# kekley/octree_pathtracing

Hardware: AMD Instinct MI355X
Metric: Mrays/sec at 1920×1080×256spp; achieved HBM GB/s vs roofline at 1/2/4/8 GPUs (higher is better)
Workload: dtype f32

## Files before the change

include/octpt.h:

```cpp
#ifndef OCTPT_H
#define OCTPT_H

#include <stddef.h>
#include <stdint.h>

#ifdef __cplusplus
extern "C" {
#endif

#define OCTPT_ABI_VERSION 4u

typedef int32_t octpt_status;
#define OCTPT_OK 0
#define OCTPT_ERR_INVALID_ARG 1
#define OCTPT_ERR_OOM 2
#define OCTPT_ERR_DEVICE 3
#define OCTPT_NOT_READY 4
#define OCTPT_ERR_UNSUPPORTED 5
#define OCTPT_CANCELLED 6
#define OCTPT_ERR_INTERNAL 7

typedef struct octpt_ctx octpt_ctx;
typedef struct octpt_frame octpt_frame;
typedef struct octpt_octree octpt_octree;
// ... 122 lines not shown
#define OCTPT_STAT_ESVO_STEPS 2
#define OCTPT_STAT_SPHERE_TESTS 3
#define OCTPT_STAT_CUBOID_TESTS 4
#define OCTPT_STAT_SHADE_EVENTS 5
#define OCTPT_STAT_TEXEL_READS 6
#define OCTPT_STAT_BLOCK_TESTS 7
#define OCTPT_STAT_ISSUED_BYTES 8
#define OCTPT_STAT_COUNT 9
typedef struct octpt_stats {
    uint64_t paths, segments, esvo_steps, sphere_tests, cuboid_tests, shade_events, texel_reads;
    uint64_t launches;
    double kernel_ms;
    uint64_t extend_launches, shade_launches;
    double extend_ms, shade_ms;
    double build_ms;
    uint64_t block_tests;
    uint64_t issued_bytes;
    uint64_t drain[OCTPT_STAT_COUNT];
    uint64_t pool_slots;
    uint64_t chunk_items;
    uint64_t wave_allocs;
    uint64_t beam_restarts;
    uint64_t hit_check_failures;
} octpt_stats;

uint32_t octpt_abi_version(void);
int32_t octpt_device_count(void);
octpt_status octpt_create(int32_t device, octpt_ctx **out);
octpt_status octpt_create_multi(const int32_t *devices, uint32_t n, octpt_ctx **out);
uint32_t octpt_device_entries(const octpt_ctx *ctx);
void octpt_destroy(octpt_ctx *ctx);
const char *octpt_last_error(const octpt_ctx *ctx);

octpt_status octpt_scene_upload(octpt_ctx *ctx, const octpt_scene_desc *scene);
octpt_status octpt_scene_build_device(octpt_ctx *ctx, const octpt_scene_desc *scene, uint32_t flags);
octpt_status octpt_set_camera(octpt_ctx *ctx, const octpt_camera *camera);
octpt_status octpt_get_camera(const octpt_ctx *ctx, octpt_camera *camera);

octpt_status octpt_render(octpt_ctx *ctx, const octpt_render_params *p, float *accum_rgba, uint8_t *out_rgba8);

octpt_status octpt_render_device(octpt_ctx *ctx, const octpt_render_params *p, float *d_accum,
                                 uint32_t *d_seg_count, void *hip_stream);

octpt_status octpt_render_async(octpt_ctx *ctx, const octpt_render_params *p, float *accum_rgba,
                                uint8_t *out_rgba8, octpt_frame **out_frame);
octpt_status octpt_frame_poll(octpt_frame *frame);
// ... 271 lines not shown
```

octree_pathtracing_amd/_lib.py:

```python
from __future__ import annotations

import ctypes as C
import os
from pathlib import Path

LIB_DIR = Path(__file__).resolve().parent / "lib"
LIB_PATH = LIB_DIR / "liboctpt.so"

OCTPT_ABI_VERSION = 4

OK = 0
ERR_INVALID_ARG = 1
ERR_OOM = 2
ERR_DEVICE = 3
NOT_READY = 4
ERR_UNSUPPORTED = 5
CANCELLED = 6
ERR_INTERNAL = 7

TEXTURE_COLOR = 0
TEXTURE_IMAGE = 1
RENDER_SHARD_COMPACT = 0x1
RENDER_MEGAKERNEL = 0x2
RENDER_KERNEL_TIMING = 0x4
# ... 210 lines not shown
    _fields_ = [("width", C.c_uint32), ("height", C.c_uint32), ("flags", C.c_uint32)]


class FinalParams(C.Structure):
    _fields_ = [("adaptive", AdaptiveParamsEx), ("filter", DenoiseVarianceParams)]


TILE = 8


STAT_NAMES = ("paths", "segments", "esvo_steps", "sphere_tests", "cuboid_tests", "shade_events", "texel_reads",
              "block_tests", "issued_bytes")
STAT_COUNT = len(STAT_NAMES)


class Stats(C.Structure):
    _fields_ = [("paths", C.c_uint64), ("segments", C.c_uint64), ("esvo_steps", C.c_uint64),
                ("sphere_tests", C.c_uint64), ("cuboid_tests", C.c_uint64), ("shade_events", C.c_uint64),
                ("texel_reads", C.c_uint64), ("launches", C.c_uint64), ("kernel_ms", C.c_double),
                ("extend_launches", C.c_uint64), ("shade_launches", C.c_uint64), ("extend_ms", C.c_double),
                ("shade_ms", C.c_double), ("build_ms", C.c_double), ("block_tests", C.c_uint64),
                ("issued_bytes", C.c_uint64), ("drain", C.c_uint64 * STAT_COUNT), ("pool_slots", C.c_uint64),
                ("chunk_items", C.c_uint64), ("wave_allocs", C.c_uint64), ("beam_restarts", C.c_uint64),
                ("hit_check_failures", C.c_uint64)]

    def as_dict(self) -> dict:
        d = {name: getattr(self, name) for name, _ in self._fields_}
        d["drain"] = dict(zip(STAT_NAMES, list(self.drain)))
        return d


class OctreeView(C.Structure):
    _fields_ = [("octants", C.c_void_p), ("octant_count", C.c_uint32), ("root", C.c_uint32), ("depth", C.c_uint32),
                ("leaf_first", C.c_void_p), ("leaf_count", C.c_void_p), ("leaf_table_size", C.c_uint32),
                ("leaf_prims", C.c_void_p), ("leaf_prim_count", C.c_uint32)]


_vp, _u32, _i32, _f = C.c_void_p, C.c_uint32, C.c_int32, C.c_float
SIGNATURES = {
    "octpt_abi_version": (_u32, []),
    "octpt_device_count": (_i32, []),
    "octpt_create": (_i32, [_i32, C.POINTER(_vp)]),
    "octpt_create_multi": (_i32, [_vp, _u32, C.POINTER(_vp)]),
    "octpt_device_entries": (_u32, [_vp]),
    "octpt_destroy": (None, [_vp]),
    "octpt_last_error": (C.c_char_p, [_vp]),
    "octpt_scene_upload": (_i32, [_vp, C.POINTER(SceneDesc)]),
# ... 109 lines not shown
```

octree_pathtracing_amd/csrc/octpt_api.cpp:

```cpp
#include <hip/hip_runtime.h>

#include <algorithm>
#include <atomic>
#include <chrono>
#include <cmath>
#include <cstdlib>
#include <thread>
#include <cstdio>
#include <cstring>
#include <new>
#include <string>
#include <memory>
#include <vector>

#include "../../include/octpt.h"
#include "octpt_internal.h"
#include "octpt_mask.h"
#include "octpt_reproject.h"

using namespace octpt;

namespace {

constexpr uint32_t kCounterRing = 256;
constexpr uint64_t kMaxChunkPaths = 1ull << 31;
constexpr uint64_t kDefaultChunkPaths = 1ull << 29;
#ifndef OCTPT_LOOKAHEAD
#define OCTPT_LOOKAHEAD 3
#endif
constexpr uint32_t kLookahead = OCTPT_LOOKAHEAD;
constexpr uint32_t kDefaultPool = 512u << 20;
constexpr uint32_t kMaxPool = 1u << 30;
constexpr uint32_t kMinPool = 1u << 20;
constexpr uint32_t kDefaultRefill = 0;
constexpr uint32_t kDefaultDrainRays = 4096;

uint32_t env_u32(const char *name, uint32_t dflt) {
    const char *v = std::getenv(name);
    if (!v || !*v) return dflt;
    const long x = std::strtol(v, nullptr, 10);
    return x > 0 ? (uint32_t)x : dflt;
}

struct EventPair {
    hipEvent_t start, stop;
};

template <class T>
struct DevBuf {
    T *p = nullptr;
    size_t n = 0;
};

}

struct octpt_ctx {
    int device = 0;
// ... 7 lines not shown
    octpt_camera cam{};
    DevCamera C{};
    uint32_t *d_counters = nullptr;
    std::vector<uint2> h_subs;
    uint2 *d_subs = nullptr;
    size_t subs_cap = 0;
    float *d_beam = nullptr;
    size_t beam_cap = 0;
    uint32_t launch_seq = 0;
    unsigned long long *d_stats = nullptr;
    uint8_t *d_lut_byte = nullptr;
    float *d_lut_float = nullptr;
    std::vector<EventPair> pending;
    double kernel_ms = 0.0;
    uint64_t launches = 0;
    bool ktiming = false;
    std::vector<std::pair<int, EventPair>> kpending;
    std::vector<EventPair> ev_pool;
    double kern_ms[2] = {0.0, 0.0};
    uint64_t kern_n[2] = {0, 0};
    float build_ms = 0.0f;
    BuildScratch build_scratch;
    int blocks_per_cu_cache[kMaxDepth + 1] = {0};
    int extend_bpc_cache[kMaxDepth + 1][4] = {};
    int shade_bpc_cache[2][2][3] = {};
    bool lean_scene = false;
    bool no_lean = false;
    WaveBuffers wb{};
    size_t pool = 0, color_cap = 0, nee_pool = 0;
    void *nee_alloc = nullptr;
    std::vector<void *> wave_allocs;
    void *color_alloc = nullptr;
    size_t wave_bytes = 0, mem_limit = 0;
    std::vector<std::pair<void *, size_t>> wave_sizes;
    uint64_t wave_allocs_n = 0;
    bool oom_warned = false;
    uint32_t *h_count = nullptr;
    uint32_t *d_count = nullptr;
    hipEvent_t count_ev[kLookahead + 1] = {};
    uint32_t pool_cap = kDefaultPool, refill = kDefaultRefill;
    bool beam = true;
    uint32_t drain_rays = kDefaultDrainRays;
    bool drain_models = false;
    uint64_t chunk_cap = kDefaultChunkPaths;
    octpt_frame *inflight = nullptr;
    std::vector<octpt_ctx *> sub;
    float4 *m_acc = nullptr;
    uint32_t *m_seg = nullptr;
    size_t m_acc_cap = 0, m_seg_cap = 0;
    float4 *dn_frame[2] = {nullptr, nullptr};
    size_t dn_cap[2] = {0, 0};
    std::vector<uint32_t> h_order;
    uint32_t order_w = 0, order_h = 0;
    uint32_t *d_order = nullptr, *d_order_pos = nullptr;
    uint64_t scene_gen = 0, camera_gen = 0, order_gen = 0;
    struct BeamKey {
        uint64_t scene = 0, camera = 0, order = 0;
        uint64_t list = 0;
        uint32_t w = 0, h = 0, shard_index = 0, shard_count = 0;
        bool valid = false;
        bool operator==(const BeamKey &o) const {
            return valid && o.valid && scene == o.scene && camera == o.camera && order == o.order && list == o.list &&
                   w == o.w && h == o.h && shard_index == o.shard_index && shard_count == o.shard_count;
// ... 742 lines not shown
                         ctx->S.sun.sun_sampling != 0, ctx->S.has_blocks != 0, &part);
        if (st == OCTPT_OK) break;
        if (st != OCTPT_ERR_OOM) return st;
        if (part == kOomColor && chunk_spp > 1 && !R.subs) {
            ctx->chunk_cap = (uint64_t)(chunk_spp / 2) * n_px;
            if (ctx->pool > ctx->chunk_cap) {
                HIP_TRY(ctx, hipDeviceSynchronize());
                free_queues(ctx);
                ctx->pool_cap = (uint32_t)std::max<uint64_t>(kMinPool, std::min<uint64_t>(ctx->pool_cap, ctx->chunk_cap));
            }
        } else if (part == kOomNee && ctx->pool > kMinPool) {
            HIP_TRY(ctx, hipDeviceSynchronize());
            ctx->pool_cap = (uint32_t)std::max<size_t>(kMinPool, ctx->pool / 2);
            free_queues(ctx);
        } else {
            return st;
        }
        if (!ctx->oom_warned)
            std::fprintf(stderr, "octpt: wavefront state did not fit in device memory; chunk %llu items, pool cap %u\n",
                         (unsigned long long)ctx->chunk_cap, ctx->pool_cap);
        ctx->oom_warned = true;
    }
    const size_t pool = (size_t)std::min<uint64_t>(std::min<uint64_t>(ctx->pool_cap, chunk_max), ctx->pool);
    int &bpc = ctx->extend_bpc_cache[ctx->S.depth][ctx->S.has_blocks ? 3 : ctx->S.has_models ? 2 : (ctx->S.has_cuboids ? 1 : 0)];
    if (bpc == 0) bpc = extend_blocks_per_cu(ctx->S);
    const int grid_extend = ctx->num_cu * bpc;
    if (std::getenv("OCTPT_DEBUG"))
        std::fprintf(stderr, "octpt: extend %d blocks/CU x %d CUs (depth %u, cuboids %u, models %u), pool %zu\n", bpc,
                     ctx->num_cu, ctx->S.depth, ctx->S.has_cuboids, ctx->S.has_models, pool);
    const int seg_blocks = (int)(kSegs * 64u / kBlock);
    const uint32_t shade_bpc_env = std::min<uint32_t>(env_u32("OCTPT_SHADE_BPC", 0u), 8u);
    auto grid_shade_of = [&](int mode) {
        int &cached = ctx->shade_bpc_cache[ctx->S.sun.sun_sampling ? 1 : 0]
                                          [shade_lds_tables(ctx->S) ? 1 : 0]
                                          [mode];
        if (cached == 0) cached = shade_blocks_per_cu(ctx->S, mode);
        const int bpc = shade_bpc_env ? (int)shade_bpc_env : cached;
        return (ctx->num_cu * bpc + seg_blocks - 1) / seg_blocks * seg_blocks;
    };
    {
        float none;
        std::memcpy(&none, &kPrimNone, sizeof none);
        ctx->wb.eye = make_float4(ctx->C.eye[0], ctx->C.eye[1], ctx->C.eye[2], none);
    }
    const WaveBuffers &B = ctx->wb;
    const float *beam = nullptr;
    if (ctx->beam) {
        const size_t n_tiles = (size_t)R.beam_tx * ((R.H + kBeamTile - 1) / kBeamTile);
        octpt_ctx::BeamKey key;
        key.scene = ctx->scene_gen;
        key.camera = ctx->camera_gen;
        key.order = ctx->order_gen;
        key.w = R.W;
        key.h = R.H;
        key.shard_index = R.shard_index;
        key.shard_count = R.shard_count;
        key.list = list;
        key.valid = true;
        if (list != 0u) {
// ... 26 lines not shown
        beam = ctx->d_beam;
    }
    for (uint32_t c0 = 0, c1 = 0; c0 < R.spp_count; c0 = c1) {
        c1 = c0 + std::min(chunk_spp, R.spp_count - c0);
        if (R.subs) {
            uint32_t e = c1;
            while (e < R.spp_count && (ctx->h_subs[e].y >> 16) != 0u) --e;
            if (e <= c0) {
                e = c1;
                while (e < R.spp_count && (ctx->h_subs[e].y >> 16) != 0u) ++e;
            }
            c1 = e;
        }
        DevRender Rc = R;
        Rc.spp_start = R.spp_start + c0;
        Rc.spp_count = c1 - c0;
        if (R.subs) Rc.subs = R.subs + c0;
        Rc.beam = beam;
        const uint32_t chunk_items = (uint32_t)((uint64_t)Rc.spp_count * n_px);
        HIP_TRY(ctx, hipMemsetAsync(B.ctrl, 0, kCtrlWords * sizeof(uint32_t), s));
        const uint32_t n_seed = (uint32_t)std::min<uint64_t>(pool, chunk_items);
        const bool regen = n_seed < chunk_items;
        ctx->wb.lean = (!regen && ctx->lean_scene && !ctx->no_lean && !R.subs) ? 1u : 0u;
        const int grid_shade = grid_shade_of(shade_mode(regen, ctx->wb.lean != 0u));
        const bool cam_rec = !regen &&((Rc.W | Rc.H) & (kTile - 1u)) == 0u;
        HIP_TRY(ctx, launch_wf_seed(ctx->C, Rc, B, n_seed, chunk_items, ctx->d_stats, s));
        for (uint32_t it = 0;; ++it) {
            if (cancel && cancel->load()) return fail(ctx, OCTPT_CANCELLED, "render cancelled");
            const uint32_t q = it & 1u;
            EventPair ev{};
            if ((st = ktimer_begin(ctx, s, ev)) != OCTPT_OK) return st;
            HIP_TRY(ctx, launch_wf_extend(ctx->S, B, q, it == 0u && cam_rec, ctx->refill, grid_extend,
                                          ctx->d_stats, s));
            if ((st = ktimer_end(ctx, s, 0, ev)) != OCTPT_OK) return st;
            if ((st = ktimer_begin(ctx, s, ev)) != OCTPT_OK) return st;
            HIP_TRY(ctx, launch_wf_shade(ctx->S, ctx->C, Rc, B, q, chunk_items, it == 0u ? (cam_rec ? 2u : 1u) : 0u,
                                         regen, grid_shade, ctx->d_stats, s));
            if ((st = ktimer_end(ctx, s, 1, ev)) != OCTPT_OK) return st;
            const uint32_t slot = it % (kLookahead + 1);
            HIP_TRY(ctx, launch_wf_snapshot(B, q ^ 1u, ctx->d_count + slot * kCountSpan, s));
            HIP_TRY(ctx, hipEventRecord(ctx->count_ev[slot], s));
            if (it >= kLookahead) {
                const uint32_t old = (it - kLookahead) % (kLookahead + 1);
                HIP_TRY(ctx, hipEventSynchronize(ctx->count_ev[old]));
                const uint32_t *h = ctx->h_count + old * kCountSpan;
                uint64_t queued = 0;
                for (uint32_t k = 0; k < kSegs; ++k) queued += h[k];
                if (queued == 0u) break;
                if (queued <= ctx->drain_rays && (!ctx->S.has_models || ctx->drain_models)) {
                    bool exhausted = true;
                    for (uint32_t k = 0; k < kSegs && exhausted; ++k) {
                        const uint32_t lo = (uint32_t)(((uint64_t)k * chunk_items) / kSegs);
                        const uint32_t hi = (uint32_t)(((uint64_t)(k + 1u) * chunk_items) / kSegs);
                        exhausted = h[kSegs + k] >= hi - lo;
                    }
                    if (exhausted) {
                        const int grid = (int)std::min<uint64_t>((queued + 3) / 4 + 1, (uint64_t)ctx->num_cu * 16u);
                        HIP_TRY(ctx, launch_wf_drain(ctx->S, Rc, B, q ^ 1u, grid, ctx->d_stats, s));
                        break;
                    }
// ... 337 lines not shown
octpt_status octpt_create(int32_t device, octpt_ctx **out) {
    if (!out) return OCTPT_ERR_INVALID_ARG;
    *out = nullptr;
    octpt_ctx *ctx = new (std::nothrow) octpt_ctx();
    if (!ctx) return OCTPT_ERR_OOM;
    auto bail = [&](octpt_status st) {
        octpt_destroy(ctx);
        return st;
    };
    int n = 0;
    if (hipGetDeviceCount(&n) != hipSuccess || n == 0) return bail(OCTPT_ERR_DEVICE);
    if (device < 0 || device >= n) return bail(OCTPT_ERR_INVALID_ARG);
    hipDeviceProp_t prop{};
    if (hipGetDeviceProperties(&prop, device) != hipSuccess) return bail(OCTPT_ERR_DEVICE);
    if (std::strncmp(prop.gcnArchName, "gfx950", 6) != 0) return bail(OCTPT_ERR_DEVICE);
    ctx->device = device;
    ctx->num_cu = prop.multiProcessorCount;
    ctx->pool_cap = std::max<uint32_t>(std::min<uint32_t>(env_u32("OCTPT_POOL", kDefaultPool), kMaxPool), 64u);
    ctx->chunk_cap = std::min<uint64_t>(env_u32("OCTPT_CHUNK", (uint32_t)kDefaultChunkPaths), kMaxChunkPaths);
    const char *refill_env = std::getenv("OCTPT_REFILL");
    ctx->refill = (refill_env && *refill_env)
                      ? std::max<uint32_t>(std::min<uint32_t>(env_u32("OCTPT_REFILL", 16u), 64u), 1u)
                      : kDefaultRefill;
    const char *drain_env = std::getenv("OCTPT_DRAIN_RAYS");
    if (drain_env && *drain_env) ctx->drain_rays = (uint32_t)std::strtoul(drain_env, nullptr, 10);
    const char *beam_env = std::getenv("OCTPT_BEAM");
    ctx->beam = !(beam_env && beam_env[0] == '0');
    const char *lean_env = std::getenv("OCTPT_LEAN");
    ctx->no_lean = lean_env && lean_env[0] == '0';
    ctx->drain_models = env_u32("OCTPT_DRAIN_MODELS", 0u) != 0u;
    ctx->mem_limit = (size_t)env_u32("OCTPT_DEVICE_MEM_LIMIT", 0u) << 20;
    if (hipSetDevice(device) != hipSuccess) return bail(OCTPT_ERR_DEVICE);
    if (hipStreamCreateWithFlags(&ctx->stream, hipStreamNonBlocking) != hipSuccess) return bail(OCTPT_ERR_DEVICE);
    if (hipMalloc(&ctx->d_counters, kCounterRing * sizeof(uint32_t)) != hipSuccess) return bail(OCTPT_ERR_OOM);
    if (hipMalloc(&ctx->d_stats, kStatWords * sizeof(unsigned long long)) != hipSuccess) return bail(OCTPT_ERR_OOM);
    if (hipMemset(ctx->d_stats, 0, kStatWords * sizeof(unsigned long long)) != hipSuccess) return bail(OCTPT_ERR_DEVICE);
    float lf[256];
    uint8_t lb[256];
    make_luts(lf, lb);
    if (hipMalloc(&ctx->d_lut_float, sizeof lf) != hipSuccess) return bail(OCTPT_ERR_OOM);
    if (hipMalloc(&ctx->d_lut_byte, sizeof lb) != hipSuccess) return bail(OCTPT_ERR_OOM);
    if (hipMemcpy(ctx->d_lut_float, lf, sizeof lf, hipMemcpyHostToDevice) != hipSuccess) return bail(OCTPT_ERR_DEVICE);
    if (hipMemcpy(ctx->d_lut_byte, lb, sizeof lb, hipMemcpyHostToDevice) != hipSuccess) return bail(OCTPT_ERR_DEVICE);
    *out = ctx;
    return OCTPT_OK;
}
// ... 1747 lines not shown
            octpt_stats cs{};
            const octpt_status st = octpt_get_stats(c, &cs);
            if (st != OCTPT_OK) return fail(ctx, st, c->err);
            tot.paths += cs.paths;
            tot.segments += cs.segments;
            tot.esvo_steps += cs.esvo_steps;
            tot.sphere_tests += cs.sphere_tests;
            tot.cuboid_tests += cs.cuboid_tests;
            tot.shade_events += cs.shade_events;
            tot.texel_reads += cs.texel_reads;
            tot.extend_launches += cs.extend_launches;
            tot.shade_launches += cs.shade_launches;
            tot.extend_ms += cs.extend_ms;
            tot.shade_ms += cs.shade_ms;
            tot.build_ms = std::max(tot.build_ms, cs.build_ms);
            tot.block_tests += cs.block_tests;
            tot.issued_bytes += cs.issued_bytes;
            for (int k = 0; k < OCTPT_STAT_COUNT; ++k) tot.drain[k] += cs.drain[k];
            tot.pool_slots = std::max(tot.pool_slots, cs.pool_slots);
            tot.chunk_items = std::max(tot.chunk_items, cs.chunk_items);
            tot.wave_allocs += cs.wave_allocs;
            tot.beam_restarts += cs.beam_restarts;
            tot.hit_check_failures += cs.hit_check_failures;
        }
        tot.build_ms = std::max(tot.build_ms, (double)ctx->build_ms);
        tot.launches = ctx->launches;
        tot.kernel_ms = ctx->kernel_ms;
        *out = tot;
        return OCTPT_OK;
    }
    HIP_TRY(ctx, hipSetDevice(ctx->device));
    for (auto &e : ctx->pending) {
        HIP_TRY(ctx, hipEventSynchronize(e.stop));
        float ms = 0.0f;
        HIP_TRY(ctx, hipEventElapsedTime(&ms, e.start, e.stop));
        ctx->kernel_ms += ms;
        (void)hipEventDestroy(e.start);
        (void)hipEventDestroy(e.stop);
    }
    ctx->pending.clear();
    for (auto &ke : ctx->kpending) {
        HIP_TRY(ctx, hipEventSynchronize(ke.second.stop));
        float ms = 0.0f;
        HIP_TRY(ctx, hipEventElapsedTime(&ms, ke.second.start, ke.second.stop));
        ctx->kern_ms[ke.first] += ms;
        ctx->kern_n[ke.first]++;
// ... 30 lines not shown
    }
    out->paths = v[kStatPaths];
    out->segments = v[kStatSegments] - redo_main;
    out->esvo_steps = v[kStatSteps];
    out->sphere_tests = v[kStatSphereTests];
    out->cuboid_tests = v[kStatCuboidTests];
    out->shade_events = v[kStatShade];
    out->texel_reads = v[kStatTexels];
    out->block_tests = v[kStatBlockTests];
    out->issued_bytes = v[kStatIssued];
    out->beam_restarts = redo_main + redo_drain;
    out->hit_check_failures = 0;
    for (uint32_t r = 0; r < 2u * kSegs; ++r) out->hit_check_failures += rows[r * kStatRow + kStatHitCheckWord];
    out->pool_slots = ctx->pool;
    out->chunk_items = ctx->color_cap;
    out->wave_allocs = ctx->wave_allocs_n;
    out->launches = ctx->launches;
    out->kernel_ms = ctx->kernel_ms;
    out->extend_launches = ctx->kern_n[0];
    out->shade_launches = ctx->kern_n[1];
    out->extend_ms = ctx->kern_ms[0];
    out->shade_ms = ctx->kern_ms[1];
    out->build_ms = ctx->build_ms;
    return OCTPT_OK;
}

octpt_status octpt_reset_stats(octpt_ctx *ctx) {
    if (!ctx) return OCTPT_ERR_INVALID_ARG;
    join_inflight(ctx);
    if (is_multi(ctx)) {
        for (octpt_ctx *c : ctx->sub) {
            const octpt_status st = octpt_reset_stats(c);
            if (st != OCTPT_OK) return fail(ctx, st, c->err);
        }
        ctx->kernel_ms = 0.0;
        ctx->launches = 0;
        return OCTPT_OK;
    }
    octpt_stats tmp;
    octpt_status st = octpt_get_stats(ctx, &tmp);
    if (st != OCTPT_OK) return st;
    HIP_TRY(ctx, hipMemset(ctx->d_stats, 0, kStatWords * sizeof(unsigned long long)));
    ctx->kernel_ms = 0.0;
    ctx->launches = 0;
    ctx->kern_ms[0] = ctx->kern_ms[1] = 0.0;
    ctx->kern_n[0] = ctx->kern_n[1] = 0;
    return OCTPT_OK;
}

octpt_status octpt_build_octree_device(octpt_ctx *ctx, const octpt_sphere *spheres, uint32_t ns,
                                       const octpt_cuboid *cuboids, uint32_t nc, uint32_t depth, octpt_octree **out) {
    return octpt_build_octree_device_ex(ctx, spheres, ns, cuboids, nc, depth, 0u, out);
}

octpt_status octpt_build_octree_device_ex(octpt_ctx *ctx, const octpt_sphere *spheres, uint32_t ns,
                                          const octpt_cuboid *cuboids, uint32_t nc, uint32_t depth, uint32_t flags,
                                          octpt_octree **out) {
    if (!ctx) return OCTPT_ERR_INVALID_ARG;
    if (!out) return fail(ctx, OCTPT_ERR_INVALID_ARG, "out NULL");
    if (flags & ~OCTPT_BUILD_COMPACT) return fail(ctx, OCTPT_ERR_INVALID_ARG, "unknown build flags");
    *out = nullptr;
    if (depth < 1 || depth > kMaxDepth) return fail(ctx, OCTPT_ERR_INVALID_ARG, "depth must be in [1, 21]");
    if ((ns && !spheres) || (nc && !cuboids)) return fail(ctx, OCTPT_ERR_INVALID_ARG, "NULL primitive array");
    return build_octree_handle(ctx, out, "octree build", [=](BuiltOctree &t, float &ms) {
        join_inflight(ctx);
        if (pair_bound(spheres, ns, cuboids, nc, depth) > kMaxBuildPairs)
            return fail(ctx, OCTPT_ERR_OOM, "more than 2^31 (cell, primitive) pairs");
        HIP_TRY(ctx, hipSetDevice(ctx->device));
        return run_prim_build(ctx, spheres, ns, cuboids, nc, depth, flags, t, nullptr, ms);
// ... 34 lines not shown
```

octree_pathtracing_amd/csrc/octpt_internal.h:

```cpp
#pragma once
#include <hip/hip_runtime.h>
#include <stdint.h>

#include <memory>
#include <new>
#include <utility>
#include <vector>

#include "../../include/octpt.h"

namespace octpt {

constexpr uint32_t kPrimNone = 0xFFFFFFFFu;
constexpr uint32_t kPrimCuboidBit = 0x80000000u;
constexpr uint32_t kPrimIndexMask = 0x07FFFFFFu;
#ifndef OCTPT_BEAM_TILE
#define OCTPT_BEAM_TILE 2
#endif
constexpr uint32_t kBeamTile = OCTPT_BEAM_TILE;
constexpr uint32_t kTile = 8;
constexpr uint32_t kBlock = 256;
constexpr uint32_t kMaxDepth = 21;
constexpr uint64_t kMaxBuildPairs = 1ull << 31;

// ... 232 lines not shown
    if (compact) {
        caller = i;
        return true;
    }
    const uint32_t t = dealt_tile(order, shard_index + u * shard_count);
    const uint32_t x = (t % tiles_x) * kTile + k % kTile, y = (t / tiles_x) * kTile + k / kTile;
    if (x >= W || y >= H) return false;
    caller = y * W + x;
    return true;
}

hipError_t launch_preview(const DevScene &S, const DevCamera &C, const DevRender &R, float4 *accum,
                          uint32_t *segcount, unsigned long long *stats, hipStream_t stream);
hipError_t launch_render(const DevScene &S, const DevCamera &C, const DevRender &R, float4 *accum,
                         uint32_t *segcount, uint32_t *counter, unsigned long long *stats, int grid,
                         hipStream_t stream);
hipError_t launch_wf_seed(const DevCamera &C, const DevRender &R, const WaveBuffers &B, uint32_t n_seed,
                          uint32_t chunk_items, unsigned long long *stats, hipStream_t stream);
hipError_t launch_wf_extend(const DevScene &S, const WaveBuffers &B, uint32_t q, bool cam, uint32_t refill, int grid,
                            unsigned long long *stats, hipStream_t stream);
hipError_t launch_wf_shade(const DevScene &S, const DevCamera &C, const DevRender &R, const WaveBuffers &B, uint32_t q,
                           uint32_t chunk_items, uint32_t first, bool regen, int grid, unsigned long long *stats,
                           hipStream_t stream);
int shade_blocks_per_cu(const DevScene &S, int mode);
bool shade_lds_tables(const DevScene &S);
hipError_t launch_wf_drain(const DevScene &S, const DevRender &R, const WaveBuffers &B, uint32_t q, int grid,
                           unsigned long long *stats, hipStream_t stream);
hipError_t launch_wf_snapshot(const WaveBuffers &B, uint32_t q, uint32_t *host_out, hipStream_t stream);
hipError_t launch_wf_resolve(const DevRender &R, const WaveBuffers &B, uint32_t chunk_spp, float4 *accum,
                             uint32_t *segcount, float2 *moments, float clamp, hipStream_t stream);
hipError_t launch_adaptive_init(uint32_t n, float4 *accum, float2 *moments, hipStream_t stream);
hipError_t launch_tile_error(uint32_t W, uint32_t H, float luminance_floor, const float2 *moments,
                             const uint32_t *tile_spp, float *error, hipStream_t stream);
hipError_t launch_tile_error_spread(uint32_t W, uint32_t H, float w, const float *error, float *out, hipStream_t stream);
hipError_t launch_sample_variance(uint32_t W, uint32_t H, const float2 *moments, const uint32_t *tile_spp,
                                  const float *depth, const float4 *albedo, float *out, hipStream_t stream);
int extend_blocks_per_cu(const DevScene &S);
hipError_t launch_intersect(const DevScene &S, const float *rays, const uint32_t *last_prim,
                            const float *last_normal, uint32_t n, float *t, uint32_t *prim, float *normal,
                            uint32_t *steps, hipStream_t stream);
hipError_t launch_beam(const DevScene &S, const DevCamera &C, const DevRender &R, float *beam, hipStream_t stream);
hipError_t launch_gbuffer(const DevScene &S, const DevCamera &C, const DevRender &R, const DevAov &out,
                          unsigned long long *stats, hipStream_t stream);
hipError_t launch_denoise_prep(uint32_t W, uint32_t H, const float4 *color, const float4 *albedo, const float *depth,
                               float4 *sig, hipStream_t stream);
hipError_t launch_atrous(const DevDenoise &D, uint32_t iter, bool last, const float4 *src, float4 *dst,
                         hipStream_t stream);
hipError_t launch_temporal(const DevTemporal &T, bool moments, hipStream_t stream);
hipError_t launch_variance(const DevVariance &V, hipStream_t stream);
hipError_t launch_denoise_var_prep(uint32_t W, uint32_t H, const float4 *color, const float *variance,
                                   const float4 *albedo, const float *depth, float4 *sig, hipStream_t stream);
hipError_t launch_atrous_var(const DevDenoiseVar &D, uint32_t iter, bool last, const float4 *src, float4 *dst,
                             hipStream_t stream);
hipError_t launch_tonemap(const float4 *accum, uchar4 *out, uint32_t n, const uint8_t *lut_byte,
                          hipStream_t stream);
hipError_t launch_unshard(uint32_t W, uint32_t H, uint32_t shard_count, const uint32_t *tile_pos, const float4 *shards,
                          uint32_t stride, float4 *frame, hipStream_t stream);
hipError_t launch_multi_stage(const DevRender &R, uint32_t n_dev, uint32_t stride, float4 *accum, uint32_t *seg,
                              float4 *stage_accum, uint32_t *stage_seg, bool to_stage, hipStream_t stream);
int render_blocks_per_cu(uint32_t depth);
// ... 91 lines not shown
```

octree_pathtracing_amd/csrc/octpt_kernels.hip:

```cpp
#include "octpt_internal.h"
#include "octpt_rcp.h"
#include "octpt_reproject.h"

#ifndef OCTPT_RCP_FAST
#define OCTPT_RCP_FAST 1
#endif

namespace octpt {
namespace {

#define RAY_EPSILON 0.00000005f
#define RAY_OFFSET 0.000001f
#define OCTREE_MAX_STEPS 1000u
#define OCTREE_MAX_SCALE 23u
#define OCTREE_EPSILON 1.1920929e-7f
#define MAX_DST_WORLD 1024.0f
#define PI_F 3.14159265358979323846f
#define CELL_TOL 0.001f
#define SUN_MAX_CHANCE 0.9f
#define MAT_FLAG_REFRACTIVE 0x4u
#define MAT_FLAG_SUBSURFACE 0x2u
#define MAX_PATH_SEGMENTS 64u
constexpr uint32_t kBeamIterBits = 10u;
constexpr uint32_t kBeamIterMask = (1u << kBeamIterBits) - 1u;
// ... 1714 lines not shown
    }
    return ok;
}

__global__ __launch_bounds__(kBlock) void wf_seed_kernel(DevCamera C, DevRender R, WaveBuffers B, uint32_t n_seed,
                                                         uint32_t chunk_items, unsigned long long *__restrict__ stats) {
    const uint32_t i = blockIdx.x * kBlock + threadIdx.x;
    const uint32_t seg = (i >> 6) % kSegs;
    Counters cnt = {0u, 0u, 0u, 0u, 0u, 0u, 0u};
    PathState ps;
    bool ok = false;
    uint32_t slot = i;
    if (n_seed == chunk_items) {
        if (blockIdx.x == 0u && threadIdx.x < kSegs)
            B.ctrl[ctr_item(threadIdx.x)] = shard_lo(threadIdx.x + 1u, chunk_items) - shard_lo(threadIdx.x, chunk_items);
        const uint32_t lo = shard_lo(seg, chunk_items), hi = shard_lo(seg + 1u, chunk_items);
        const uint32_t item = lo + (i >> 6) / kSegs * 64u + (i & 63u);
        slot = item;
        if (item < hi) ok = seed_item<true>(C, R, B, slot, item, ps, cnt);
        if (((R.W | R.H) & (kTile - 1u)) == 0u) {
            if (blockIdx.x == 0u && threadIdx.x < kSegs)
                B.ctrl[ctr_count(0u, threadIdx.x)] = shard_lo(threadIdx.x + 1u, chunk_items) - shard_lo(threadIdx.x, chunk_items);
            if (ok) store_cam_ray(B, seg * B.seg_cap + (item - lo), ps);
            if (blockIdx.x == 0u && threadIdx.x == 0u) B.ray0[0][0] = B.eye;
            if (blockIdx.x == 0u && threadIdx.x == 0u) atomicAdd(&stats[kStatPaths], (unsigned long long)chunk_items);
            return;
        }
    } else {
        ItemCursor cur = {seg, true};
        ok = regen<true>(C, R, B, i, i < n_seed, chunk_items, cur, ps, cnt);
    }
    const uint32_t t = wave_ticket(B.ctrl + ctr_count(0u, seg), ok);
    if (ok) store_ray(B, 0u, seg * B.seg_cap + t, slot, ps);
    flush_counters(cnt, stats);
}

#ifndef OCTPT_SPH_WAVES
#define OCTPT_SPH_WAVES 8
#endif
#ifndef OCTPT_BOX_WAVES
#define OCTPT_BOX_WAVES 7
#endif
#ifndef OCTPT_MDL_WAVES
#define OCTPT_MDL_WAVES 6
#endif
#ifndef OCTPT_BLK_WAVES
#define OCTPT_BLK_WAVES 6
#endif
#define OCTPT_EXTEND_WAVES_OF(k)                                                                              \
    ((k) == kPrimsSpheres ? OCTPT_SPH_WAVES                                                                   \
                          : (k) == kPrimsBoxes ? OCTPT_BOX_WAVES : (k) == kPrimsBlocks ? OCTPT_BLK_WAVES : OCTPT_MDL_WAVES)
#ifndef OCTPT_CLAIM
#define OCTPT_CLAIM 64
#endif
constexpr uint32_t kClaim = OCTPT_CLAIM;
static_assert(kSegs % 8u == 0u, "eight XCDs share the segments evenly");
#ifndef OCTPT_THR_LONG
#define OCTPT_THR_LONG 16
#endif
#ifndef OCTPT_THR_SHORT
#define OCTPT_THR_SHORT 32
#endif
#ifndef OCTPT_SHORT_STEPS
#define OCTPT_SHORT_STEPS 48
#endif
constexpr uint32_t kShortRaySteps = OCTPT_SHORT_STEPS;
template <int kPrims>
__global__ __launch_bounds__(kBlock, OCTPT_EXTEND_WAVES_OF(kPrims)) void wf_extend_kernel(DevScene S, WaveBuffers B, uint32_t q, uint32_t refill,
                                                           unsigned long long *__restrict__ stats) {
    extern __shared__ uint2 lds_stack[];
    const Stack stk = stack_of(lds_stack, S.depth);
    const float4 *ray0 = B.ray0[q], *ray1 = B.ray1[q];
    const bool cam = (refill >> 31) != 0u;
    refill &= 0x7FFFFFFFu;
    if (blockIdx.x == 0 && threadIdx.x < kSegs) {
        B.ctrl[ctr_count(q ^ 1u, threadIdx.x)] = 0u;
        B.ctrl[ctr_head(q ^ 1u, threadIdx.x)] = 0u;
    }
    uint32_t seg = __builtin_amdgcn_readfirstlane(((blockIdx.x * kBlock + threadIdx.x) >> 6) % kSegs);
    uint32_t seg_n = B.ctrl[ctr_count(q, seg)];
    if constexpr (kPrims == kPrimsModels) seg_n = __builtin_amdgcn_readfirstlane(seg_n);
    bool rays_left = true;
    uint32_t segs_w = 0u;
    Counters cnt = {0u, 0u, 0u, 0u, 0u, 0u, 0u};
    constexpr uint32_t kIdle = 8u;
    uint32_t pos = 0u;
    TraceRay tr;
    Esvo E;
    E.idx = kIdle;
    bool more = true;
    const uint32_t lane = threadIdx.x & 63u;
    uint32_t c_next = 0u, c_end = 0u, claim_v = 0u;
    uint32_t thr = refill ? refill : OCTPT_THR_LONG;
    if (lane == 0u)
        claim_v = __hip_atomic_fetch_add(B.ctrl + ctr_head(q, seg), kClaim, __ATOMIC_RELAXED, __HIP_MEMORY_SCOPE_AGENT);
    do {
        const bool idle = E.idx >= kIdle;
        const uint64_t im = __ballot(idle);
        if (rays_left && (uint32_t)__popcll(im) >= thr) {
            if (c_next >= c_end) {
                c_next = __builtin_amdgcn_readfirstlane(claim_v);
                c_end = c_next < seg_n ? __builtin_amdgcn_readfirstlane(min(c_next + kClaim, seg_n))
                                       : c_next;
                if (c_next >= c_end) {
                    uint32_t j = lane;
                    if constexpr (kPrims != kPrimsSpheres) asm volatile("" : "+v"(j));
                    const uint64_t m = __ballot(relaxed_load(B.ctrl + ctr_head(q, j)) < B.ctrl[ctr_count(q, j)]);
                    rays_left = m != 0ull;
                    if (rays_left) {
                        seg = __builtin_amdgcn_readfirstlane(first_from(m, seg));
                        seg_n = B.ctrl[ctr_count(q, seg)];
                        if constexpr (kPrims == kPrimsModels) seg_n = __builtin_amdgcn_readfirstlane(seg_n);
                    }
                }
                if (rays_left && lane == 0u)
                    claim_v = __hip_atomic_fetch_add(B.ctrl + ctr_head(q, seg), kClaim,
                                                     __ATOMIC_RELAXED, __HIP_MEMORY_SCOPE_AGENT);
            }
            const uint32_t avail = c_end - c_next;
            if (idle) {
                const uint32_t r = lanes_below(im);
                if (r < avail) {
                    pos = seg * B.seg_cap + c_next + r;
                    const float4 r1 = ray1[pos];
                    const float4 r0 = ray0[cam ? 0u : pos];
                    const float bm = cam ? r1.w : ray_beam(r0, r1);
                    tr = make_trace_ray(S, V(r0.x, r0.y, r0.z), V(r1.x, r1.y, r1.z), ray_last_prim(r0, r1),
                                        (__float_as_uint(r1.w) >> 31) != 0u);
                    esvo_begin(S, tr, E, stk, bm);
                    cnt.steps -= E.iter;
                }
            }
            const uint32_t took = min((uint32_t)__popcll(im), avail);
            segs_w += took;
            c_next += took;
            if (refill == 0u) {
                const bool short_rays = (int64_t)(int32_t)cnt.steps * 64 < (int64_t)kShortRaySteps * segs_w;
                thr = __popcll(__ballot(short_rays)) > 32 ? OCTPT_THR_SHORT : OCTPT_THR_LONG;
            }
        }
        const uint32_t stop_at = __builtin_amdgcn_readfirstlane(rays_left ? thr : 64u);
        if ((uint32_t)__popcll(__ballot(E.idx >= kIdle)) < stop_at) do {
#ifdef OCTPT_PROFILE_LANES
            prof_wave(cnt.p_iters, cnt.p_active, E.idx < kIdle);
#endif
            if (E.idx < kIdle) {
                uint32_t prim = kPrimNone;
#ifndef OCTPT_CHECK_HITS
                if constexpr (kPrims != kPrimsModels) asm("" : "=v"(prim));
#endif
                PrimHit h;
                HIT_POISON(prim, h);
// ... 1011 lines not shown
    if (D.out_variance) D.out_variance[p] = o.w;
    const float alpha = D.color[p].w;
    if (D.albedo && zp != __builtin_inff()) {
        const float4 a = D.albedo[p];
        o.x = o.x * fmaxf(a.x, kDnAlbedoFloor);
        o.y = o.y * fmaxf(a.y, kDnAlbedoFloor);
        o.z = o.z * fmaxf(a.z, kDnAlbedoFloor);
    }
    D.out[p] = make_float4(o.x, o.y, o.z, alpha);
}

}

size_t render_lds_bytes(uint32_t depth) { return (size_t)(depth - 1u) * kBlock * (sizeof(uint2) + sizeof(uint16_t)); }

int render_blocks_per_cu(uint32_t depth) {
    int blocks = 0;
    if (hipOccupancyMaxActiveBlocksPerMultiprocessor(&blocks, reinterpret_cast<const void *>(render_kernel<true, kPrimsModels>),
                                                     kBlock, render_lds_bytes(depth)) != hipSuccess)
        return 1;
    return blocks > 0 ? blocks : 1;
}

static const void *extend_instance(const DevScene &S) {
    if (S.has_blocks) return reinterpret_cast<const void *>(wf_extend_kernel<kPrimsBlocks>);
    if (S.has_models) return reinterpret_cast<const void *>(wf_extend_kernel<kPrimsModels>);
    if (S.has_cuboids) return reinterpret_cast<const void *>(wf_extend_kernel<kPrimsBoxes>);
    return reinterpret_cast<const void *>(wf_extend_kernel<kPrimsSpheres>);
}

int extend_blocks_per_cu(const DevScene &S) {
    int blocks = 0;
    if (hipOccupancyMaxActiveBlocksPerMultiprocessor(&blocks, extend_instance(S), kBlock, render_lds_bytes(S.depth)) !=
        hipSuccess)
        return 1;
    return blocks > 0 ? blocks : 1;
}

hipError_t launch_preview(const DevScene &S0, const DevCamera &C, const DevRender &R, float4 *accum,
                          uint32_t *segcount, unsigned long long *stats, hipStream_t stream) {
    const DevScene &S = S0;
    const uint32_t grid = (R.total_items + kBlock - 1u) / kBlock;
    const void *fn = S.has_blocks   ? reinterpret_cast<const void *>(preview_kernel<kPrimsBlocks>)
                     : S.has_models ? reinterpret_cast<const void *>(preview_kernel<kPrimsModels>)
                     : S.has_cuboids ? reinterpret_cast<const void *>(preview_kernel<kPrimsBoxes>)
                                     : reinterpret_cast<const void *>(preview_kernel<kPrimsSpheres>);
    void *args[] = {const_cast<DevScene *>(&S), const_cast<DevCamera *>(&C), const_cast<DevRender *>(&R), &accum,
                    &segcount, &stats};
    const hipError_t e = hipLaunchKernel(fn, dim3(grid), dim3(kBlock), args,
                                         render_lds_bytes(S.depth), stream);
    if (e != hipSuccess) return e;
    return hipGetLastError();
}

hipError_t launch_gbuffer(const DevScene &S, const DevCamera &C, const DevRender &R, const DevAov &out,
                          unsigned long long *stats, hipStream_t stream) {
    const uint32_t grid = (R.total_items + kBlock - 1u) / kBlock;
// ... 52 lines not shown

hipError_t launch_render(const DevScene &S0, const DevCamera &C, const DevRender &R, float4 *accum, uint32_t *segcount,
                         uint32_t *counter, unsigned long long *stats, int grid, hipStream_t stream) {
    const DevScene &S = S0;
    auto kern = S.sun.sun_sampling ? (S.has_blocks ? render_kernel<true, kPrimsBlocks> : render_kernel<true, kPrimsModels>)
                                   : (S.has_blocks ? render_kernel<false, kPrimsBlocks> : render_kernel<false, kPrimsModels>);
    hipLaunchKernelGGL(kern, dim3(grid), dim3(kBlock), render_lds_bytes(S.depth), stream, S, C, R, accum, segcount,
                       counter, stats);
    return hipGetLastError();
}

hipError_t launch_wf_seed(const DevCamera &C, const DevRender &R, const WaveBuffers &B, uint32_t n_seed,
                          uint32_t chunk_items, unsigned long long *stats, hipStream_t stream) {
    const uint64_t threads = n_seed == chunk_items
                                 ? (uint64_t)kSegs * ((((uint64_t)chunk_items + kSegs - 1u) / kSegs + 63u) / 64u) * 64u
                                 : (uint64_t)n_seed;
    hipLaunchKernelGGL(wf_seed_kernel, dim3((uint32_t)((threads + kBlock - 1u) / kBlock)), dim3(kBlock), 0, stream, C, R, B, n_seed,
                       chunk_items, stats);
    return hipGetLastError();
}

hipError_t launch_wf_extend(const DevScene &S, const WaveBuffers &B, uint32_t q, bool cam, uint32_t refill, int grid,
                            unsigned long long *stats, hipStream_t stream) {
    uint32_t rf = refill | (cam ? 0x80000000u : 0u);
    void *args[] = {const_cast<DevScene *>(&S), const_cast<WaveBuffers *>(&B), &q, &rf, &stats};
    const hipError_t e = hipLaunchKernel(extend_instance(S), dim3(grid), dim3(kBlock), args, render_lds_bytes(S.depth),
                                         stream);
    if (e != hipSuccess) return e;
    return hipGetLastError();
}

template <bool kLds, int kSP>
static const void *lean_shade_of(bool first) {
    return !first ? reinterpret_cast<const void *>(wf_shade_kernel<false, kLds, 2, true, kSP>)
                  : reinterpret_cast<const void *>(wf_shade_kernel<false, kLds, 2, false, kSP>);
}
template <bool kNee, bool kLds>
static const void *shade_instance_of(int mode, bool first, int prims) {
    if (!kNee && mode == 2) {
        if (prims == kShadeSphColour) return lean_shade_of<kLds, kShadeSphColour>(first);
        if (prims == kPrimsSpheres) return lean_shade_of<kLds, kPrimsSpheres>(first);
        if (prims == kPrimsBoxes) return lean_shade_of<kLds, kPrimsBoxes>(first);
        if (prims == kPrimsBlocks) return lean_shade_of<kLds, kPrimsBlocks>(first);
        return lean_shade_of<kLds, kPrimsModels>(first);
    }
    return mode == 1 ? reinterpret_cast<const void *>(wf_shade_kernel<kNee, kLds, 1>)
                     : reinterpret_cast<const void *>(wf_shade_kernel<kNee, kLds, 0>);
}
bool shade_lds_tables(const DevScene &S) { return S.n_mats <= kShadeLdsMats && S.n_texs <= kShadeLdsMats; }
static const void *shade_instance(const DevScene &S, int mode, bool first = false) {
    const bool lds = shade_lds_tables(S);
    const int prims = S.has_blocks    ? kPrimsBlocks
                      : S.has_models  ? kPrimsModels
                      : S.has_cuboids ? kPrimsBoxes
                      : S.has_images  ? kPrimsSpheres
                                      : kShadeSphColour;
    return S.sun.sun_sampling
               ? (lds ? shade_instance_of<true, true>(mode, first, prims) : shade_instance_of<true, false>(mode, first, prims))
               : (lds ? shade_instance_of<false, true>(mode, first, prims) : shade_instance_of<false, false>(mode, first, prims));
}

int shade_blocks_per_cu(const DevScene &S, int mode) {
    int blocks = 0;
    if (hipOccupancyMaxActiveBlocksPerMultiprocessor(&blocks, shade_instance(S, mode), kBlock, 0) != hipSuccess)
        return 4;
    return blocks > 0 ? blocks : 1;
}

hipError_t launch_wf_shade(const DevScene &S, const DevCamera &C, const DevRender &R, const WaveBuffers &B, uint32_t q,
                           uint32_t chunk_items, uint32_t first, bool regen, int grid, unsigned long long *stats,
                           hipStream_t stream) {
    uint32_t first_u = first;
    void *args[] = {const_cast<DevScene *>(&S), const_cast<DevCamera *>(&C), const_cast<DevRender *>(&R),
                    const_cast<WaveBuffers *>(&B), &q, &chunk_items, &first_u, &stats};
    const hipError_t e = hipLaunchKernel(shade_instance(S, shade_mode(regen, B.lean != 0u), first != 0u), dim3(grid),
                                         dim3(kBlock), args, 0, stream);
    if (e != hipSuccess) return e;
    return hipGetLastError();
}

hipError_t launch_wf_drain(const DevScene &S, const DevRender &R, const WaveBuffers &B, uint32_t q, int grid,
                           unsigned long long *stats, hipStream_t stream) {
    const bool nee = S.sun.sun_sampling != 0;
    const void *fn = S.has_blocks ? (nee ? reinterpret_cast<const void *>(wf_drain_kernel<kPrimsBlocks, true>)
                                         : reinterpret_cast<const void *>(wf_drain_kernel<kPrimsBlocks, false>))
                     : S.has_models ? (nee ? reinterpret_cast<const void *>(wf_drain_kernel<kPrimsModels, true>)
                                         : reinterpret_cast<const void *>(wf_drain_kernel<kPrimsModels, false>))
// ... 106 lines not shown
```

Before: 5149.

## Specialize extend kernel for camera rays with uniform origin and refill

```diff
diff --git a/include/octpt.h b/include/octpt.h
--- a/include/octpt.h
+++ b/include/octpt.h
@@ -168,6 +168,7 @@
     uint64_t wave_allocs;
     uint64_t beam_restarts;
     uint64_t hit_check_failures;
+    uint64_t extend_cam_launches;
 } octpt_stats;
 
 uint32_t octpt_abi_version(void);
diff --git a/octree_pathtracing_amd/_lib.py b/octree_pathtracing_amd/_lib.py
--- a/octree_pathtracing_amd/_lib.py
+++ b/octree_pathtracing_amd/_lib.py
@@ -256,7 +256,7 @@
                 ("shade_ms", C.c_double), ("build_ms", C.c_double), ("block_tests", C.c_uint64),
                 ("issued_bytes", C.c_uint64), ("drain", C.c_uint64 * STAT_COUNT), ("pool_slots", C.c_uint64),
                 ("chunk_items", C.c_uint64), ("wave_allocs", C.c_uint64), ("beam_restarts", C.c_uint64),
-                ("hit_check_failures", C.c_uint64)]
+                ("hit_check_failures", C.c_uint64), ("extend_cam_launches", C.c_uint64)]
 
     def as_dict(self) -> dict:
         d = {name: getattr(self, name) for name, _ in self._fields_}
diff --git a/octree_pathtracing_amd/csrc/octpt_api.cpp b/octree_pathtracing_amd/csrc/octpt_api.cpp
--- a/octree_pathtracing_amd/csrc/octpt_api.cpp
+++ b/octree_pathtracing_amd/csrc/octpt_api.cpp
@@ -33,6 +33,8 @@
 constexpr uint32_t kMaxPool = 1u << 30;
 constexpr uint32_t kMinPool = 1u << 20;
 constexpr uint32_t kDefaultRefill = 0;
+constexpr uint32_t kSphereCamRefill = 16;
+constexpr uint32_t kRefillCamUnset = 0xFFFFFFFFu;
 constexpr uint32_t kDefaultDrainRays = 4096;
 
 uint32_t env_u32(const char *name, uint32_t dflt) {
@@ -86,8 +88,9 @@
     float build_ms = 0.0f;
     BuildScratch build_scratch;
     int blocks_per_cu_cache[kMaxDepth + 1] = {0};
-    int extend_bpc_cache[kMaxDepth + 1][4] = {};
-    int shade_bpc_cache[2][2][3] = {};
+    int extend_bpc_cache[kMaxDepth + 1][4][2] = {};
+    int shade_bpc_cache[2][2][3][kShadePrimKinds][2] = {};
+    uint64_t extend_cam_n = 0;
     bool lean_scene = false;
     bool no_lean = false;
     WaveBuffers wb{};
@@ -103,6 +106,7 @@
     uint32_t *d_count = nullptr;
     hipEvent_t count_ev[kLookahead + 1] = {};
     uint32_t pool_cap = kDefaultPool, refill = kDefaultRefill;
+    uint32_t refill_cam = kRefillCamUnset;
     bool beam = true;
     uint32_t drain_rays = kDefaultDrainRays;
     bool drain_models = false;
@@ -891,19 +895,27 @@
         ctx->oom_warned = true;
     }
     const size_t pool = (size_t)std::min<uint64_t>(std::min<uint64_t>(ctx->pool_cap, chunk_max), ctx->pool);
-    int &bpc = ctx->extend_bpc_cache[ctx->S.depth][ctx->S.has_blocks ? 3 : ctx->S.has_models ? 2 : (ctx->S.has_cuboids ? 1 : 0)];
-    if (bpc == 0) bpc = extend_blocks_per_cu(ctx->S);
-    const int grid_extend = ctx->num_cu * bpc;
+    auto grid_extend_of = [&](bool cam) {
+        int &bpc = ctx->extend_bpc_cache[ctx->S.depth]
+                                        [ctx->S.has_blocks ? 3 : ctx->S.has_models ? 2 : (ctx->S.has_cuboids ? 1 : 0)]
+                                        [cam ? 1 : 0];
+        if (bpc == 0) bpc = extend_blocks_per_cu(ctx->S, cam);
+        return ctx->num_cu * bpc;
+    };
+    const int grid_extend = grid_extend_of(false);
     if (std::getenv("OCTPT_DEBUG"))
-        std::fprintf(stderr, "octpt: extend %d blocks/CU x %d CUs (depth %u, cuboids %u, models %u), pool %zu\n", bpc,
-                     ctx->num_cu, ctx->S.depth, ctx->S.has_cuboids, ctx->S.has_models, pool);
+        std::fprintf(stderr, "octpt: extend %d blocks/CU (camera records: %d) x %d CUs (depth %u, cuboids %u, models %u), "
+                             "pool %zu\n", grid_extend / ctx->num_cu, grid_extend_of(true) / ctx->num_cu, ctx->num_cu,
+                     ctx->S.depth, ctx->S.has_cuboids, ctx->S.has_models, pool);
     const int seg_blocks = (int)(kSegs * 64u / kBlock);
     const uint32_t shade_bpc_env = std::min<uint32_t>(env_u32("OCTPT_SHADE_BPC", 0u), 8u);
-    auto grid_shade_of = [&](int mode) {
+    auto grid_shade_of = [&](int mode, bool first) {
         int &cached = ctx->shade_bpc_cache[ctx->S.sun.sun_sampling ? 1 : 0]
                                           [shade_lds_tables(ctx->S) ? 1 : 0]
-                                          [mode];
-        if (cached == 0) cached = shade_blocks_per_cu(ctx->S, mode);
+                                          [mode]
+                                          [shade_prims(ctx->S)]
+                                          [first ? 1 : 0];
+        if (cached == 0) cached = shade_blocks_per_cu(ctx->S, mode, first);
         const int bpc = shade_bpc_env ? (int)shade_bpc_env : cached;
         return (ctx->num_cu * bpc + seg_blocks - 1) / seg_blocks * seg_blocks;
     };
@@ -976,7 +988,8 @@
         const uint32_t n_seed = (uint32_t)std::min<uint64_t>(pool, chunk_items);
         const bool regen = n_seed < chunk_items;
         ctx->wb.lean = (!regen && ctx->lean_scene && !ctx->no_lean && !R.subs) ? 1u : 0u;
-        const int grid_shade = grid_shade_of(shade_mode(regen, ctx->wb.lean != 0u));
+        const int mode = shade_mode(regen, ctx->wb.lean != 0u);
+        const int grid_shade = grid_shade_of(mode, false), grid_shade_first = grid_shade_of(mode, true);
         const bool cam_rec = !regen &&((Rc.W | Rc.H) & (kTile - 1u)) == 0u;
         HIP_TRY(ctx, launch_wf_seed(ctx->C, Rc, B, n_seed, chunk_items, ctx->d_stats, s));
         for (uint32_t it = 0;; ++it) {
@@ -984,12 +997,18 @@
             const uint32_t q = it & 1u;
             EventPair ev{};
             if ((st = ktimer_begin(ctx, s, ev)) != OCTPT_OK) return st;
-            HIP_TRY(ctx, launch_wf_extend(ctx->S, B, q, it == 0u && cam_rec, ctx->refill, grid_extend,
-                                          ctx->d_stats, s));
+            const bool cam = it == 0u && cam_rec;
+            const bool spheres_only = !ctx->S.has_blocks && !ctx->S.has_models && !ctx->S.has_cuboids;
+            const uint32_t refill_cam = ctx->refill_cam != kRefillCamUnset ? ctx->refill_cam
+                                        : spheres_only                     ? kSphereCamRefill
+                                                                           : kDefaultRefill;
+            HIP_TRY(ctx, launch_wf_extend(ctx->S, B, q, cam, cam ? refill_cam : ctx->refill,
+                                          cam ? grid_extend_of(true) : grid_extend, ctx->d_stats, s));
+            ctx->extend_cam_n += cam ? 1u : 0u;
             if ((st = ktimer_end(ctx, s, 0, ev)) != OCTPT_OK) return st;
             if ((st = ktimer_begin(ctx, s, ev)) != OCTPT_OK) return st;
             HIP_TRY(ctx, launch_wf_shade(ctx->S, ctx->C, Rc, B, q, chunk_items, it == 0u ? (cam_rec ? 2u : 1u) : 0u,
-                                         regen, grid_shade, ctx->d_stats, s));
+                                         regen, it == 0u ? grid_shade_first : grid_shade, ctx->d_stats, s));
             if ((st = ktimer_end(ctx, s, 1, ev)) != OCTPT_OK) return st;
             const uint32_t slot = it % (kLookahead + 1);
             HIP_TRY(ctx, launch_wf_snapshot(B, q ^ 1u, ctx->d_count + slot * kCountSpan, s));
@@ -1373,6 +1392,10 @@
     ctx->refill = (refill_env && *refill_env)
                       ? std::max<uint32_t>(std::min<uint32_t>(env_u32("OCTPT_REFILL", 16u), 64u), 1u)
                       : kDefaultRefill;
+    const char *refill_cam_env = std::getenv("OCTPT_REFILL_CAM");
+    ctx->refill_cam = (refill_env && *refill_env) ? ctx->refill
+                      : (refill_cam_env && *refill_cam_env) ? std::min<uint32_t>(env_u32("OCTPT_REFILL_CAM", 16u), 64u)
+                                                            : kRefillCamUnset;
     const char *drain_env = std::getenv("OCTPT_DRAIN_RAYS");
     if (drain_env && *drain_env) ctx->drain_rays = (uint32_t)std::strtoul(drain_env, nullptr, 10);
     const char *beam_env = std::getenv("OCTPT_BEAM");
@@ -3166,6 +3189,7 @@
             tot.wave_allocs += cs.wave_allocs;
             tot.beam_restarts += cs.beam_restarts;
             tot.hit_check_failures += cs.hit_check_failures;
+            tot.extend_cam_launches += cs.extend_cam_launches;
         }
         tot.build_ms = std::max(tot.build_ms, (double)ctx->build_ms);
         tot.launches = ctx->launches;
@@ -3242,6 +3266,7 @@
     out->extend_ms = ctx->kern_ms[0];
     out->shade_ms = ctx->kern_ms[1];
     out->build_ms = ctx->build_ms;
+    out->extend_cam_launches = ctx->extend_cam_n;
     return OCTPT_OK;
 }
 
@@ -3265,6 +3290,7 @@
     ctx->launches = 0;
     ctx->kern_ms[0] = ctx->kern_ms[1] = 0.0;
     ctx->kern_n[0] = ctx->kern_n[1] = 0;
+    ctx->extend_cam_n = 0;
     return OCTPT_OK;
 }
 
diff --git a/octree_pathtracing_amd/csrc/octpt_internal.h b/octree_pathtracing_amd/csrc/octpt_internal.h
--- a/octree_pathtracing_amd/csrc/octpt_internal.h
+++ b/octree_pathtracing_amd/csrc/octpt_internal.h
@@ -278,7 +278,9 @@
 hipError_t launch_wf_shade(const DevScene &S, const DevCamera &C, const DevRender &R, const WaveBuffers &B, uint32_t q,
                            uint32_t chunk_items, uint32_t first, bool regen, int grid, unsigned long long *stats,
                            hipStream_t stream);
-int shade_blocks_per_cu(const DevScene &S, int mode);
+int shade_blocks_per_cu(const DevScene &S, int mode, bool first);
+constexpr int kShadePrimKinds = 5;
+int shade_prims(const DevScene &S);
 bool shade_lds_tables(const DevScene &S);
 hipError_t launch_wf_drain(const DevScene &S, const DevRender &R, const WaveBuffers &B, uint32_t q, int grid,
                            unsigned long long *stats, hipStream_t stream);
@@ -291,7 +293,7 @@
 hipError_t launch_tile_error_spread(uint32_t W, uint32_t H, float w, const float *error, float *out, hipStream_t stream);
 hipError_t launch_sample_variance(uint32_t W, uint32_t H, const float2 *moments, const uint32_t *tile_spp,
                                   const float *depth, const float4 *albedo, float *out, hipStream_t stream);
-int extend_blocks_per_cu(const DevScene &S);
+int extend_blocks_per_cu(const DevScene &S, bool cam);
 hipError_t launch_intersect(const DevScene &S, const float *rays, const uint32_t *last_prim,
                             const float *last_normal, uint32_t n, float *t, uint32_t *prim, float *normal,
                             uint32_t *steps, hipStream_t stream);
diff --git a/octree_pathtracing_amd/csrc/octpt_kernels.hip b/octree_pathtracing_amd/csrc/octpt_kernels.hip
--- a/octree_pathtracing_amd/csrc/octpt_kernels.hip
+++ b/octree_pathtracing_amd/csrc/octpt_kernels.hip
@@ -1760,7 +1760,6 @@
             if (blockIdx.x == 0u && threadIdx.x < kSegs)
                 B.ctrl[ctr_count(0u, threadIdx.x)] = shard_lo(threadIdx.x + 1u, chunk_items) - shard_lo(threadIdx.x, chunk_items);
             if (ok) store_cam_ray(B, seg * B.seg_cap + (item - lo), ps);
-            if (blockIdx.x == 0u && threadIdx.x == 0u) B.ray0[0][0] = B.eye;
             if (blockIdx.x == 0u && threadIdx.x == 0u) atomicAdd(&stats[kStatPaths], (unsigned long long)chunk_items);
             return;
         }
@@ -1803,14 +1802,12 @@
 #define OCTPT_SHORT_STEPS 48
 #endif
 constexpr uint32_t kShortRaySteps = OCTPT_SHORT_STEPS;
-template <int kPrims>
+template <int kPrims, bool kCam>
 __global__ __launch_bounds__(kBlock, OCTPT_EXTEND_WAVES_OF(kPrims)) void wf_extend_kernel(DevScene S, WaveBuffers B, uint32_t q, uint32_t refill,
                                                            unsigned long long *__restrict__ stats) {
     extern __shared__ uint2 lds_stack[];
     const Stack stk = stack_of(lds_stack, S.depth);
     const float4 *ray0 = B.ray0[q], *ray1 = B.ray1[q];
-    const bool cam = (refill >> 31) != 0u;
-    refill &= 0x7FFFFFFFu;
     if (blockIdx.x == 0 && threadIdx.x < kSegs) {
         B.ctrl[ctr_count(q ^ 1u, threadIdx.x)] = 0u;
         B.ctrl[ctr_head(q ^ 1u, threadIdx.x)] = 0u;
@@ -1824,6 +1821,7 @@
     constexpr uint32_t kIdle = 8u;
     uint32_t pos = 0u;
     TraceRay tr;
+    if constexpr (kCam) tr = make_trace_ray(S, V(B.eye.x, B.eye.y, B.eye.z), V(0.0f, 0.0f, 0.0f), kPrimNone, false);
     Esvo E;
     E.idx = kIdle;
     bool more = true;
@@ -1861,11 +1859,20 @@
                 if (r < avail) {
                     pos = seg * B.seg_cap + c_next + r;
                     const float4 r1 = ray1[pos];
-                    const float4 r0 = ray0[cam ? 0u : pos];
-                    const float bm = cam ? r1.w : ray_beam(r0, r1);
-                    tr = make_trace_ray(S, V(r0.x, r0.y, r0.z), V(r1.x, r1.y, r1.z), ray_last_prim(r0, r1),
-                                        (__float_as_uint(r1.w) >> 31) != 0u);
-                    esvo_begin(S, tr, E, stk, bm);
+                    float bm;
+                    if constexpr (kCam) {
+                        tr.d = V(r1.x, r1.y, r1.z);
+                        bm = r1.w;
+                        TraceRay tb = tr;
+                        asm volatile("" : "+s"(tb.o.x), "+s"(tb.o.y), "+s"(tb.o.z));
+                        esvo_begin(S, tb, E, stk, bm);
+                    } else {
+                        const float4 r0 = ray0[pos];
+                        bm = ray_beam(r0, r1);
+                        tr = make_trace_ray(S, V(r0.x, r0.y, r0.z), V(r1.x, r1.y, r1.z), ray_last_prim(r0, r1),
+                                            (__float_as_uint(r1.w) >> 31) != 0u);
+                        esvo_begin(S, tr, E, stk, bm);
+                    }
                     cnt.steps -= E.iter;
                 }
             }
@@ -2923,17 +2930,21 @@
     return blocks > 0 ? blocks : 1;
 }
 
-static const void *extend_instance(const DevScene &S) {
-    if (S.has_blocks) return reinterpret_cast<const void *>(wf_extend_kernel<kPrimsBlocks>);
-    if (S.has_models) return reinterpret_cast<const void *>(wf_extend_kernel<kPrimsModels>);
-    if (S.has_cuboids) return reinterpret_cast<const void *>(wf_extend_kernel<kPrimsBoxes>);
-    return reinterpret_cast<const void *>(wf_extend_kernel<kPrimsSpheres>);
-}
-
-int extend_blocks_per_cu(const DevScene &S) {
+template <bool kCam>
+static const void *extend_instance_of(const DevScene &S) {
+    if (S.has_blocks) return reinterpret_cast<const void *>(wf_extend_kernel<kPrimsBlocks, kCam>);
+    if (S.has_models) return reinterpret_cast<const void *>(wf_extend_kernel<kPrimsModels, kCam>);
+    if (S.has_cuboids) return reinterpret_cast<const void *>(wf_extend_kernel<kPrimsBoxes, kCam>);
+    return reinterpret_cast<const void *>(wf_extend_kernel<kPrimsSpheres, kCam>);
+}
+static const void *extend_instance(const DevScene &S, bool cam) {
+    return cam ? extend_instance_of<true>(S) : extend_instance_of<false>(S);
+}
+
+int extend_blocks_per_cu(const DevScene &S, bool cam) {
     int blocks = 0;
-    if (hipOccupancyMaxActiveBlocksPerMultiprocessor(&blocks, extend_instance(S), kBlock, render_lds_bytes(S.depth)) !=
-        hipSuccess)
+    if (hipOccupancyMaxActiveBlocksPerMultiprocessor(&blocks, extend_instance(S, cam), kBlock,
+                                                     render_lds_bytes(S.depth)) != hipSuccess)
         return 1;
     return blocks > 0 ? blocks : 1;
 }
@@ -3032,10 +3043,9 @@
 
 hipError_t launch_wf_extend(const DevScene &S, const WaveBuffers &B, uint32_t q, bool cam, uint32_t refill, int grid,
                             unsigned long long *stats, hipStream_t stream) {
-    uint32_t rf = refill | (cam ? 0x80000000u : 0u);
-    void *args[] = {const_cast<DevScene *>(&S), const_cast<WaveBuffers *>(&B), &q, &rf, &stats};
-    const hipError_t e = hipLaunchKernel(extend_instance(S), dim3(grid), dim3(kBlock), args, render_lds_bytes(S.depth),
-                                         stream);
+    void *args[] = {const_cast<DevScene *>(&S), const_cast<WaveBuffers *>(&B), &q, &refill, &stats};
+    const hipError_t e = hipLaunchKernel(extend_instance(S, cam), dim3(grid), dim3(kBlock), args,
+                                         render_lds_bytes(S.depth), stream);
     if (e != hipSuccess) return e;
     return hipGetLastError();
 }
@@ -3058,21 +3068,29 @@
                      : reinterpret_cast<const void *>(wf_shade_kernel<kNee, kLds, 0>);
 }
 bool shade_lds_tables(const DevScene &S) { return S.n_mats <= kShadeLdsMats && S.n_texs <= kShadeLdsMats; }
+int shade_prims(const DevScene &S) {
+    static_assert(kPrimsSpheres >= 0 && kPrimsBoxes >= 0 && kPrimsModels >= 0 && kPrimsBlocks >= 0 &&
+                      kPrimsSpheres < kShadePrimKinds && kPrimsBoxes < kShadePrimKinds &&
+                      kPrimsModels < kShadePrimKinds && kPrimsBlocks < kShadePrimKinds &&
+                      kShadeSphColour < kShadePrimKinds,
+                  "shade_prims indexes the host's occupancy table");
+    return S.has_blocks    ? kPrimsBlocks
+           : S.has_models  ? kPrimsModels
+           : S.has_cuboids ? kPrimsBoxes
+           : S.has_images  ? kPrimsSpheres
+                           : kShadeSphColour;
+}
 static const void *shade_instance(const DevScene &S, int mode, bool first = false) {
     const bool lds = shade_lds_tables(S);
-    const int prims = S.has_blocks    ? kPrimsBlocks
-                      : S.has_models  ? kPrimsModels
-                      : S.has_cuboids ? kPrimsBoxes
-                      : S.has_images  ? kPrimsSpheres
-                                      : kShadeSphColour;
+    const int prims = shade_prims(S);
     return S.sun.sun_sampling
                ? (lds ? shade_instance_of<true, true>(mode, first, prims) : shade_instance_of<true, false>(mode, first, prims))
                : (lds ? shade_instance_of<false, true>(mode, first, prims) : shade_instance_of<false, false>(mode, first, prims));
 }
 
-int shade_blocks_per_cu(const DevScene &S, int mode) {
+int shade_blocks_per_cu(const DevScene &S, int mode, bool first) {
     int blocks = 0;
-    if (hipOccupancyMaxActiveBlocksPerMultiprocessor(&blocks, shade_instance(S, mode), kBlock, 0) != hipSuccess)
+    if (hipOccupancyMaxActiveBlocksPerMultiprocessor(&blocks, shade_instance(S, mode, first), kBlock, 0) != hipSuccess)
         return 4;
     return blocks > 0 ? blocks : 1;
 }
```

Result: no change. 5189 (median of 6 runs) (+0.8%).
